# ChainSafe/halo2-verifier

Measured on AMD Instinct MI355X. Metric: proofs verified/sec (BN254, k=14), higher is better.
Workload: dtype u32 limbs (254-bit prime-field integers)

## Files before the change

halo2_verifier_amd/csrc/batch.h:

```cpp
#pragma once
#include "ctx.h"
#include "vkplan.h"
#include <algorithm>
#include <memory>

namespace h2v {

#define H2V_DEV_ST_INVALID_INSTANCES (-40)
#define H2V_DEV_ST_TRANSCRIPT (-30)
#define H2V_DEV_ST_PANIC (-20)
#define H2V_DEV_ST_OPENING (-10)
__device__ __forceinline__ void status_set(int* status, uint32_t p, int dev_code) { atomicMin(&status[p], dev_code); }
__device__ __forceinline__ int status_get(const int* status, uint32_t p) { return __hip_atomic_load(&status[p], __ATOMIC_RELAXED, __HIP_MEMORY_SCOPE_AGENT); }
inline int status_decode(int dev) {
    switch (dev) {
        case 0: return 0;
        case H2V_DEV_ST_INVALID_INSTANCES: return H2V_ERR_INVALID_INSTANCES;
        case H2V_DEV_ST_TRANSCRIPT: return H2V_ERR_TRANSCRIPT;
        case H2V_DEV_ST_PANIC: return H2V_ERR_REFERENCE_PANIC;
        case H2V_DEV_ST_OPENING: return H2V_ERR_OPENING;
        default: return dev;
    }
}

// ... 7 lines not shown
    const Fr* chal; const Fr* mult;
    int* status;
    uint32_t* msm_scal; uint32_t np;
    Fr* shared;
    uint32_t* left_scal;
    const Fr* insteval;
    uint32_t* guard_scal; uint32_t n_guard;
    const VmInstr* code_k[3][FRVM_MAX_STREAMS] = {{nullptr}}; uint32_t n_code_k[3][FRVM_MAX_STREAMS] = {{0}}; uint32_t n_slots_k[3] = {0, 0, 0};
    uint32_t streams = 0;
    int force_streams = 0, force_lds_kb = 0;
};

struct InstEvalArgs {
    const uint8_t* inst; uint32_t ninst;
    const Fr* chal; uint32_t x_chal;
    uint32_t n, k;
    uint32_t base, len;
    Fr w_start, omega, omega_step, omega_step_inv, n_inv;
    Fr* out;
    int* status;
};
int instance_eval_enqueue(hipStream_t s, const InstEvalArgs& a);

inline uint32_t stream_words_for(size_t stream_len, int transcript) {
    const uint32_t words = (uint32_t)((stream_len + 7) / 8);
    const uint32_t blockw = transcript == H2V_TRANSCRIPT_KECCAK256 ? 17 : 16;
    return (words + blockw) / blockw * blockw;
}
struct StageArgs {
    uint32_t n;
    const Plan* plan; const PlanDevice* pd;
    const uint8_t* proofs; const uint8_t* inst;
    G1A* pts; G1A* phi; uint8_t* ycanon; int* status;
    unsigned long long* words; uint32_t stream_words;
    Fr* chal;
};

int decompress_begin_enqueue(hipStream_t s, const StageArgs& g);
int decompress_range_enqueue(hipStream_t s, const StageArgs& g, uint32_t p0, uint32_t p1);
int decompress_finish_enqueue(hipStream_t s, const StageArgs& g);
int transcript_stage_enqueue(hipStream_t s, const StageArgs& g);
size_t multipliers_scratch(uint32_t n_tail, uint32_t groups);
int multipliers_enqueue(hipStream_t s, const uint8_t* d_tail, uint32_t n_tail, uint32_t n, uint32_t groups, Fr* d_mult, Fr* d_scratch);
size_t ragged_multipliers_tiles(uint32_t n);
int ragged_multipliers_enqueue(hipStream_t s, const uint8_t* d_tail, const uint8_t* d_last, uint32_t n, Fr* d_mult, Fr* d_tile_prod, uint32_t* d_tile_words);
int leg_weights_enqueue(hipStream_t s, const uint8_t* d_tail, const Fr* d_mult, const uint32_t* d_off, uint32_t gs, uint32_t groups, uint32_t* d_weights, uint32_t* d_legs);
int gather_multipliers_enqueue(hipStream_t s, const Fr* d_src, const uint32_t* d_idx, uint32_t n, Fr* d_out);
int frvm_enqueue(hipStream_t s, const FrvmArgs& a, uint32_t n_slots);
int fold_shared_enqueue(hipStream_t s, const Fr* d_shared, uint32_t n, uint32_t np, uint32_t n_shared, uint32_t groups, uint32_t* d_msm_scal);
int fold_shared_offsets_enqueue(hipStream_t s, const Fr* d_shared, uint32_t n, uint32_t np, uint32_t n_shared, uint32_t groups, const uint32_t* d_off, uint32_t* d_msm_scal);
struct FoldRange {
    const Fr* shared;
    uint32_t n, n_shared;
    uint32_t first, count;
    uint32_t out, pad;
};
int fold_shared_ranges_enqueue(hipStream_t s, const FoldRange* d_ranges, uint32_t n_ranges, uint32_t max_shared, uint32_t* d_out);

struct Recheck {
    MsmWorkspace ws;
    DevBuf<FoldRange> ranges;
    DevBuf<uint32_t> fold;
    DevBuf<G1J> acc;
    DevBuf<uint32_t> ok;
// ... 104 lines not shown
```

halo2_verifier_amd/csrc/batch.hip:

```cpp
#include "../../include/h2v.h"
#include "batch.h"
#include <string.h>
#include <algorithm>
#include <utility>
#include <stdio.h>

using namespace h2v;

namespace h2v {

struct BatchSizes {
    uint32_t stream_words;
    size_t proofs, inst, pts, ycanon, words, chal, mult, slots, msm_scal, shared, left_scal, insteval, guard_scal, acc, results;
    uint32_t ws_terms, ws_problems, ws_per_problem;
};
BatchSizes batch_sizes(const Plan& pl, size_t N, size_t G, size_t largest) {
    BatchSizes z;
    z.stream_words = stream_words_for(pl.stream.size(), pl.opts.transcript);
    z.proofs = N * pl.proof_len;
    z.inst = N * (size_t)pl.n_instance_values * 32;
    z.pts = N * pl.n_points + pl.n_shared;
    z.ycanon = N * pl.n_points * 32;
    z.words = (size_t)z.stream_words * N;
    z.chal = (size_t)pl.squeeze_at.size() * N;
    z.mult = N;
    z.slots = (size_t)std::max(std::max(pl.n_slots, pl.n_slots_k[0]), std::max(pl.n_slots_k[1], pl.n_slots_k[2])) * N;
    z.msm_scal = (N * pl.n_points + G * pl.n_shared) * 8;
    z.shared = (size_t)pl.n_shared * N;
    z.left_scal = N * pl.n_points * 8;
    z.insteval = N * pl.inst_queries.size();
    z.guard_scal = N * pl.guard_term_order.size() * 8;
    z.acc = 2 * G;
    z.results = ResultsLayout{G, N}.total();
    z.ws_terms = (uint32_t)(2 * (N * pl.n_points + G * pl.n_shared));
    z.ws_problems = (uint32_t)(2 * G);
    z.ws_per_problem = (uint32_t)(largest * pl.n_points + pl.n_shared);
    return z;
}

int ensure_buffers(h2v_batch* b, const Plan& pl) {
    const size_t N = b->max_proofs, G = b->groups;
    size_t largest = (N + G - 1) / G;
    if (ragged(b)) { largest = 0; for (size_t g = 0; g < G; ++g) largest = std::max<size_t>(largest, b->group_off[g + 1] - b->group_off[g]); }
    const BatchSizes z = batch_sizes(pl, N, G, largest);
    int rc;
    if ((rc = b->proofs.reserve(z.proofs)) || (rc = b->inst.reserve(z.inst)) || (rc = b->pts.reserve(z.pts)) || (rc = b->phi.reserve(z.pts)) ||
// ... 265 lines not shown
    return 0;
}

int launch_impl(h2v_batch* b, int with_pairing, const Fr* ext_mult, const uint32_t* ext_idx) {
    int rc;
    if ((rc = require_stage(b, BatchStage::Uploaded, "h2v_batch_launch"))) return rc;
    StageCommit commit{b};
    h2v_ctx* ctx = b->ctx;
    H2V_HIP_CHECK(hipSetDevice(ctx->device));
    PlanDevice* pd = b->plan;
    const Plan& pl = pd->host;
    hipStream_t s = b->stream;
    uint32_t n = b->n;
    const uint32_t G = b->groups;
    if ((rc = join_tail(b))) return rc;
    int ev = 0;
    auto mark = [&]() { if (b->profiling >= 2) hipEventRecord(b->ev[ev], s); ++ev; };
    mark();
    const StageArgs g = stage_args(b);
    const bool run_decompress = !(b->stage == BatchStage::Uploaded && b->decompressed);
    const ResultsLayout L{G, n};
    if (run_decompress && n) H2V_HIP_CHECK(hipMemsetAsync(b->fold_failed, 0, L.total() - L.fold_failed(), s));
    else H2V_HIP_CHECK(hipMemsetAsync(b->fold_failed, 0, 4 * (size_t)G, s));
    if (run_decompress && n && ((rc = decompress_finish_enqueue(s, g)) || (rc = decompress_range_enqueue(s, g, 0, n)))) return rc;
    mark();
    if ((rc = transcript_stage_enqueue(s, g))) return rc;
    MsmProblems pr;
    for (uint32_t g = 0; g < G; ++g)
        channel_problems(pr, b, pl, group_first(b, g), (uint32_t)group_count(b, g), b->acc.p + 2 * g, b->msm_scal.p + ((size_t)n * pl.n_points + (size_t)g * pl.n_shared) * 8, n ? pl.n_shared : 0);
    b->ws.tune = ctx->tuning;
    if (n) {
        if (ext_mult) { b->mult_of_draws = false; if ((rc = gather_multipliers_enqueue(s, ext_mult, ext_idx, n, b->mult.p))) return rc; }
        else if (!b->mult_of_draws) { if ((rc = draw_multipliers_enqueue(b))) return rc; b->mult_of_draws = true; }
        if (!(pl.left_term_order.size() == 1 && !pl.left_term_order[0].first)) H2V_HIP_CHECK(hipMemsetAsync(b->left_scal.p, 0, (size_t)n * pl.n_points * 32, s));
    }
    mark();
    FrvmArgs a{pd->code.p, (uint32_t)pl.code.size(), pd->consts.p, b->slots.p, n, b->proofs.p, pl.proof_len, pd->scalar_offsets.p, b->inst.p, pl.n_instance_values,
               b->chal.p, b->mult.p, b->status, b->msm_scal.p, pl.n_points, b->shared.p, b->left_scal.p, b->insteval.p, b->guard_scal.p, (uint32_t)pl.guard_term_order.size()};
    if (n && pl.wide_instances) {
        Fr step = pl.omega;
        for (int i = 0; i < 8; ++i) step = step.sqr();
        const Fr step_inv = step.inv();
        for (size_t q = 0; q < pl.inst_queries.size(); ++q) {
            InstEvalArgs ia{b->inst.p, pl.n_instance_values, b->chal.p, pl.x_chal, n, pl.domain_k, pl.inst_queries[q].base, pl.inst_queries[q].len,
                            pl.inst_queries[q].w_start, pl.omega, step, step_inv, pl.n_inv, b->insteval.p + q * (size_t)n, b->status};
            if ((rc = instance_eval_enqueue(s, ia))) return rc;
        }
    }
    a.force_streams = ctx->tuning.frvm_streams; a.force_lds_kb = ctx->tuning.frvm_lds_kb;
// ... 408 lines not shown
```

halo2_verifier_amd/csrc/verify_kernels.hip:

```cpp
#include "../../include/h2v.h"
#include "batch.h"
#include <atomic>

namespace h2v {

#define K_DECOMPRESS_LDS_WORDS 2560
__global__ void __launch_bounds__(64, 4) k_decompress(const uint8_t* __restrict__ proofs, uint32_t proof_len, const uint32_t* __restrict__ point_offsets,
                                                   uint32_t np, uint32_t n_main_points, uint32_t n, G1A* __restrict__ pts, G1A* __restrict__ phi, uint8_t* __restrict__ ycanon,
                                                   int* __restrict__ status) {
    const uint32_t t_raw = blockIdx.x * blockDim.x + threadIdx.x;
    const uint32_t t = min(t_raw, n * np - 1);
    uint32_t p = t / np, slot = t % np;
    const uint4* src = reinterpret_cast<const uint4*>(proofs + (size_t)p * proof_len + point_offsets[slot]);
    const uint4 lo = src[0], hi = src[1];
    uint32_t w[8] = {lo.x, lo.y, lo.z, lo.w, hi.x, hi.y, hi.z, hi.w};
    const bool is_inf = (w[7] >> 24) & G1_FLAG_IDENTITY, sign = (w[7] >> 24) & G1_FLAG_SIGN;
    w[7] &= 0x3fffffffu;
    G1A a = G1A::identity();
    bool ok = !Fq::geq_p(w);
    uint32_t yraw[8] = {0, 0, 0, 0, 0, 0, 0, 0};
    if (ok) {
        const Fq x = Fq::from_raw(w);
        if (is_inf) ok = false;
        else {
            const Fq three = {{FqParams::ONE(0), FqParams::ONE(1), FqParams::ONE(2), FqParams::ONE(3), FqParams::ONE(4), FqParams::ONE(5), FqParams::ONE(6), FqParams::ONE(7), FqParams::ONE(8)}};
            const Fq rhs = x.sqr() * x + (three + three + three);
            Fq y = fq_sqrt_candidate_loop_w3(rhs);
            if (y.sqr() != rhs) ok = false;
            else {
                y.to_raw(yraw);
                uint32_t nz = 0;
#pragma unroll
// ... 20 lines not shown
    for (int i = 0; i < 18; ++i) { const uint32_t k = i * 64 + lane; if (k < live * 18) dp[k] = out_lds[k]; }
    __syncthreads();
    a.x = g1_beta_times(a.x);
#pragma unroll
    for (int i = 0; i < 9; ++i) out_lds[lane * 18 + i] = av[i];
    __syncthreads();
    dp = reinterpret_cast<uint32_t*>(phi + t0);
#pragma unroll
    for (int i = 0; i < 18; ++i) { const uint32_t k = i * 64 + lane; if (k < live * 18) dp[k] = out_lds[k]; }
    __syncthreads();
#pragma unroll
    for (int i = 0; i < 8; ++i) out_lds[lane * 8 + i] = yraw[i];
    __syncthreads();
    uint32_t* dy = reinterpret_cast<uint32_t*>(ycanon + (size_t)t0 * 32);
#pragma unroll
    for (int i = 0; i < 8; ++i) { const uint32_t k = i * 64 + lane; if (k < live * 8) dy[k] = out_lds[k]; }
}

__global__ void __launch_bounds__(256) k_check_scalars(const uint8_t* __restrict__ proofs, uint32_t proof_len, const uint32_t* __restrict__ scalar_offsets,
                                                       uint32_t ns, const uint8_t* __restrict__ inst, uint32_t ninst, uint32_t n, int* __restrict__ status) {
    uint32_t t = blockIdx.x * blockDim.x + threadIdx.x;
    uint32_t per = ns + ninst;
    if (t >= n * per) return;
    uint32_t p = t / per, i = t % per;
    const uint8_t* b = i < ns ? proofs + (size_t)p * proof_len + scalar_offsets[i] : inst + ((size_t)p * ninst + (i - ns)) * 32;
    const uint32_t top = ((uintptr_t)b & 3u) == 0 ? *reinterpret_cast<const uint32_t*>(b + 28)
                                                  : (uint32_t)b[28] | ((uint32_t)b[29] << 8) | ((uint32_t)b[30] << 16) | ((uint32_t)b[31] << 24);
    if (top < FrParams::P(7)) return;
    uint32_t raw[8];
    for (int j = 0; j < 8; ++j) raw[j] = (uint32_t)b[4 * j] | ((uint32_t)b[4 * j + 1] << 8) | ((uint32_t)b[4 * j + 2] << 16) | ((uint32_t)b[4 * j + 3] << 24);
    if (Fr::geq_p(raw)) status_set(status, p, i < ns ? H2V_DEV_ST_TRANSCRIPT : H2V_DEV_ST_INVALID_INSTANCES);
}

#define STREAM_PROOFS_PER_BLOCK 8u
__global__ void __launch_bounds__(256) k_stream_build(const TranscriptSrc* __restrict__ stream, uint32_t stream_len, const uint8_t* __restrict__ proofs,
                                                      uint32_t proof_len, const uint8_t* __restrict__ ycanon, uint32_t np, const uint8_t* __restrict__ inst,
                                                      uint32_t ninst, uint32_t n, uint32_t stream_words, unsigned long long* __restrict__ words) {
    const uint32_t p0 = blockIdx.x * STREAM_PROOFS_PER_BLOCK, p1 = min(n, p0 + STREAM_PROOFS_PER_BLOCK);
    for (uint32_t w = threadIdx.x; w < stream_words; w += blockDim.x) {
        uint32_t kind[8], value[8], off[8];
#pragma unroll
        for (uint32_t b = 0; b < 8; ++b) {
            const uint32_t pos = w * 8 + b, q = pos < stream_len ? pos : stream_len - 1;
            const TranscriptSrc sd = stream[q];
            kind[b] = pos < stream_len ? sd.kind : (uint32_t)TranscriptSrc::CONST;
            value[b] = pos < stream_len ? sd.value : 0u;
            off[b] = kind[b] == TranscriptSrc::CONST ? 0u : sd.offset;
        }
        auto is_data = [](uint32_t k) { return k != TranscriptSrc::CONST; };
        auto src_of = [](uint32_t k) { return k == TranscriptSrc::PROOF_MASKED ? (uint32_t)TranscriptSrc::PROOF : k; };
        uint32_t la = 0;
        while (la < 8 && is_data(kind[la]) && src_of(kind[la]) == src_of(kind[0]) && off[la] == off[0] + la) ++la;
        uint32_t sb = la;
        unsigned long long cbytes = 0;
// ... 127 lines not shown
        }
        const uint32_t rem = len - last_blk * 128;
        __syncthreads();
#pragma unroll
        for (uint32_t j = 0; j < 4; ++j) {
            unsigned long long w = pf_blk == last_blk ? pf[j] : words[(size_t)last_blk * 16 + 4 * r + j];
            const uint32_t lo = 8 * (4 * r + j);
            if (lo >= rem) w = 0;
            else if (lo + 8 > rem) w &= (1ULL << (8 * (rem - lo))) - 1;
            msg[4 * r + j] = w;
        }
        __syncthreads();
        unsigned long long c0 = h0, c1 = h1;
        blake2b_compress_quad(c0, c1, msg, sig, len, true, r);
        dig[q * 8 + r] = c0; dig[q * 8 + 4 + r] = c1;
    }
    __syncthreads();
    for (uint32_t q = r; q < n_squeeze; q += 4) {
        uint32_t w32[16];
#pragma unroll
        for (int i = 0; i < 8; ++i) { const unsigned long long v = dig[q * 8 + i]; w32[2 * i] = (uint32_t)v; w32[2 * i + 1] = (uint32_t)(v >> 32); }
        const Fr c = Fr::from_uniform_words(w32);
        if (p_raw < n) chal[(size_t)q * n + p] = c;
    }
}

__device__ __forceinline__ unsigned long long rotl64(unsigned long long x, int c) { return c ? (x << c) | (x >> (64 - c)) : x; }
__constant__ unsigned long long KECCAK_RC[24] = {
    0x0000000000000001ULL, 0x0000000000008082ULL, 0x800000000000808aULL, 0x8000000080008000ULL, 0x000000000000808bULL, 0x0000000080000001ULL,
    0x8000000080008081ULL, 0x8000000000008009ULL, 0x000000000000008aULL, 0x0000000000000088ULL, 0x0000000080008009ULL, 0x000000008000000aULL,
    0x000000008000808bULL, 0x800000000000008bULL, 0x8000000000008089ULL, 0x8000000000008003ULL, 0x8000000000008002ULL, 0x8000000000000080ULL,
    0x000000000000800aULL, 0x800000008000000aULL, 0x8000000080008081ULL, 0x8000000000008080ULL, 0x0000000080000001ULL, 0x8000000080008008ULL};
__device__ __noinline__ void keccak_f1600(unsigned long long a[25]) {
    const int ROT[25] = {0, 1, 62, 28, 27, 36, 44, 6, 55, 20, 3, 10, 43, 25, 39, 41, 45, 15, 21, 8, 18, 2, 61, 56, 14};
    for (int r = 0; r < 24; ++r) {
        unsigned long long c[5], b[25];
#pragma unroll
        for (int x = 0; x < 5; ++x) c[x] = a[x] ^ a[x + 5] ^ a[x + 10] ^ a[x + 15] ^ a[x + 20];
#pragma unroll
        for (int x = 0; x < 5; ++x) {
            unsigned long long d = c[(x + 4) % 5] ^ rotl64(c[(x + 1) % 5], 1);
#pragma unroll
            for (int y = 0; y < 5; ++y) a[x + 5 * y] ^= d;
        }
#pragma unroll
        for (int x = 0; x < 5; ++x)
// ... 393 lines not shown
    red[t] = acc;
    __syncthreads();
    for (uint32_t d = 32; d > 0; d >>= 1) {
        if (t < d) red[t] = red[t] + red[t + d];
        __syncthreads();
    }
    if (t == 0) {
        uint32_t raw[8]; red[0].to_raw(raw);
        uint32_t* dst = out + ((size_t)rg.out + j) * 8;
        for (int i = 0; i < 8; ++i) dst[i] = raw[i];
    }
}

int decompress_begin_enqueue(hipStream_t s, const StageArgs& g) {
    if (g.n) H2V_HIP_CHECK(hipMemsetAsync(g.status, 0, sizeof(int) * g.n, s));
    return 0;
}
int decompress_range_enqueue(hipStream_t s, const StageArgs& g, uint32_t p0, uint32_t p1) {
    if (p1 <= p0) return 0;
    const Plan& pl = *g.plan;
    const uint32_t m = p1 - p0, tp = m * pl.n_points;
    if (!tp) return 0;
    hipLaunchKernelGGL(k_decompress, dim3((tp + 63) / 64), dim3(64), 0, s, g.proofs + (size_t)p0 * pl.proof_len, pl.proof_len, g.pd->point_offsets.p, pl.n_points, pl.n_main_points, m,
                       g.pts + (size_t)p0 * pl.n_points, g.phi + (size_t)p0 * pl.n_points, g.ycanon + (size_t)p0 * pl.n_points * 32, g.status + p0);
    H2V_HIP_CHECK(hipGetLastError());
    return 0;
}
int decompress_finish_enqueue(hipStream_t s, const StageArgs& g) {
    const Plan& pl = *g.plan;
    const uint32_t ts = g.n * (pl.n_scalars + pl.n_instance_values);
    if (ts) hipLaunchKernelGGL(k_check_scalars, dim3((ts + 255) / 256), dim3(256), 0, s, g.proofs, pl.proof_len, g.pd->scalar_offsets.p, pl.n_scalars, g.inst, pl.n_instance_values, g.n, g.status);
    H2V_HIP_CHECK(hipGetLastError());
    return 0;
}
int transcript_stage_enqueue(hipStream_t s, const StageArgs& g) {
    const uint32_t n = g.n;
    if (!n) return 0;
    const Plan& pl = *g.plan;
    uint32_t stream_len = (uint32_t)pl.stream.size();
    uint32_t n_words = g.stream_words;
    const bool keccak = pl.opts.transcript == H2V_TRANSCRIPT_KECCAK256;
    const uint32_t nsq = (uint32_t)pl.squeeze_at.size();
    const size_t lds = ((size_t)16 * TR4_MSG_STRIDE + (size_t)16 * nsq * 8) * 8;
    if (!keccak && lds > 60 * 1024) { set_last_error("transcript: too many challenges for one workgroup's LDS"); return H2V_ERR_UNSUPPORTED; }
    hipLaunchKernelGGL(k_stream_build, dim3((n + STREAM_PROOFS_PER_BLOCK - 1) / STREAM_PROOFS_PER_BLOCK), dim3(256), 0, s, g.pd->stream.p, stream_len, g.proofs, pl.proof_len, g.ycanon, pl.n_points, g.inst,
                       pl.n_instance_values, n, n_words, g.words);
    if (keccak)
        hipLaunchKernelGGL(k_transcript_keccak, dim3((n + 63) / 64), dim3(64), 0, s, g.words, n_words, g.pd->squeeze_at.p, nsq, n, g.chal);
    else
        hipLaunchKernelGGL(k_transcript, dim3((n + 15) / 16), dim3(64), lds, s, g.words, n_words, g.pd->squeeze_at.p, nsq, n, g.chal);
    H2V_HIP_CHECK(hipGetLastError());
    return 0;
}
size_t multipliers_scratch(uint32_t n_tail, uint32_t groups) { return (size_t)groups * ((n_tail / groups + MULT_TILE - 1) / MULT_TILE); }
int multipliers_enqueue(hipStream_t s, const uint8_t* d_tail, uint32_t n_tail, uint32_t n, uint32_t groups, Fr* d_mult, Fr* d_scratch) {
    const uint32_t nt = n_tail / groups, ng = n / groups, tiles = (nt + MULT_TILE - 1) / MULT_TILE;
    if (!tiles || !ng) return 0;
    if (tiles > 65535u * 1024u || groups > 65535u) { set_last_error("multipliers: too many draws or groups"); return H2V_ERR_BAD_ARGUMENT; }
    hipLaunchKernelGGL(k_mult_tiles, dim3(tiles, groups), dim3(MULT_TILE), 0, s, d_tail, nt, ng, tiles, d_mult, d_scratch);
    if (tiles > 1) {
        hipLaunchKernelGGL(k_mult_scan_tiles, dim3(groups), dim3(1024), 0, s, d_scratch, tiles);
        hipLaunchKernelGGL(k_mult_apply, dim3((ng + MULT_TILE - 1) / MULT_TILE, groups), dim3(MULT_TILE), 0, s, d_mult, ng, tiles, (const Fr*)d_scratch);
    }
    H2V_HIP_CHECK(hipGetLastError());
    return 0;
}
size_t ragged_multipliers_tiles(uint32_t n) { return ((size_t)n + MULT_TILE - 1) / MULT_TILE; }
int ragged_multipliers_enqueue(hipStream_t s, const uint8_t* d_tail, const uint8_t* d_last, uint32_t n, Fr* d_mult, Fr* d_tile_prod, uint32_t* d_tile_words) {
    const uint32_t tiles = (uint32_t)ragged_multipliers_tiles(n);
    if (!tiles) return 0;
    uint32_t* tile_closed = d_tile_words; uint32_t* open_from = d_tile_words + tiles;
    hipLaunchKernelGGL(k_seg_mult_tiles, dim3(tiles), dim3(MULT_TILE), 0, s, d_tail, d_last, n, d_mult, d_tile_prod, tile_closed, open_from);
    if (tiles > 1) {
// ... 75 lines not shown
```

halo2_verifier_amd/csrc/vkplan.h:

```cpp
#pragma once
#include "ctx.h"
#include <map>
#include <mutex>

namespace h2v {

static const uint8_t COL_INSTANCE = 254, COL_FIXED = 255;
struct ColumnH { uint32_t index; uint8_t type; };
struct QueryH { ColumnH column; int32_t rotation; };
struct TermH { uint16_t coeff_idx; std::vector<std::pair<uint32_t, uint32_t>> factors; };
struct ExprH { uint32_t num_vars = 0; std::vector<TermH> terms; };
struct LookupH { std::vector<ExprH> input, table; };
struct ShuffleH { std::vector<ExprH> input, shuffle; };

struct VkHost {
    uint32_t k = 0, cs_degree = 0;
    std::vector<G1A> fixed_commitments, permutation_commitments;
    Fr transcript_repr;
    uint32_t num_fixed_columns = 0, num_advice_columns = 0, num_instance_columns = 0, num_selectors = 0, num_challenges = 0;
    std::vector<uint8_t> advice_column_phase, challenge_phase;
    std::vector<uint32_t> num_advice_queries;
    std::vector<QueryH> advice_queries, instance_queries, fixed_queries;
    std::vector<ColumnH> permutation_columns;
    std::vector<ExprH> gates;
// ... 16 lines not shown
    OP_INV = 6,
    OP_POW = 7,
    OP_SQRN = 8,
    OP_LOAD_SCALAR = 9,
    OP_LOAD_INST = 10,
    OP_LOAD_CHAL = 11,
    OP_LOAD_MULT = 12,
    OP_STORE_MSM = 13,
    OP_STORE_SHARED = 14,
    OP_STORE_LEFT = 15,
    OP_LOAD_INSTEVAL = 16,
    OP_STORE_GUARD = 17,
    OP_BARRIER = 18,
};
struct VmInstr { uint32_t op, d, a, b; };
#define FRVM_MAX_STREAMS 4
#define VM_CONST_OPERAND 0x80000000u

struct TranscriptSrc {
    enum Kind : uint8_t { CONST = 0, PROOF = 1, PROOF_MASKED = 2, YCOORD = 3, INSTANCE = 4 };
    uint8_t kind; uint8_t value; uint32_t offset;
};

struct PlanOptions { int multiopen = 0; int transcript = 0; int circuit_instances = 1; bool guard_terms = false; int instance_kernel_threshold = 0; };

struct Plan {
    PlanOptions opts;
    double dag_work = 0, dag_critical_path = 0, makespan_k[3] = {0, 0, 0};
    uint32_t n_points = 0, n_scalars = 0, proof_len = 0;
    std::vector<uint32_t> point_offsets, scalar_offsets;
    uint32_t n_main_points = 0;
    uint32_t slot_h1 = 0, slot_h2 = 0;
    uint32_t opening_offset = 0;
    std::vector<std::pair<uint8_t, uint32_t>> left_term_order;
    std::vector<TranscriptSrc> stream;
    std::vector<uint32_t> squeeze_at;
    std::vector<uint32_t> squeeze_order;
    uint32_t n_challenges = 0;
    uint32_t n_user_challenges = 0;
    std::vector<VmInstr> code;
    std::vector<Fr> consts;
    uint32_t n_slots = 0;
    std::vector<VmInstr> code_k[3][FRVM_MAX_STREAMS];
    uint32_t n_slots_k[3] = {0, 0, 0};
    uint32_t n_shared = 0;
    std::vector<G1A> shared_bases;
    std::vector<std::pair<uint8_t, uint32_t>> right_term_order;
    std::vector<std::pair<uint8_t, uint32_t>> guard_term_order;
    std::vector<size_t> col_lens;
    uint32_t n_instance_values = 0;
    struct InstQuery { uint32_t base, len; Fr w_start; };
    bool wide_instances = false;
    std::vector<InstQuery> inst_queries;
    uint32_t x_chal = 0, domain_k = 0;
    Fr omega, n_inv;
};
int compile_plan(const VkHost& vk, const ParamsHost& params, const std::vector<size_t>& col_lens, PlanOptions opts, Plan& out, std::string& err);

struct PlanDevice {
    Plan host;
    DevBuf<VmInstr> code;
    DevBuf<VmInstr> code_k[3][FRVM_MAX_STREAMS];
    DevBuf<Fr> consts;
    DevBuf<TranscriptSrc> stream;
    DevBuf<uint32_t> squeeze_at;
    DevBuf<uint32_t> point_offsets;
    DevBuf<uint32_t> scalar_offsets;
    DevBuf<G1A> shared_bases, shared_phi;
    int pins = 0;
    uint64_t last_use = 0;
    int upload();
};

#define H2V_MAX_CACHED_PLANS 32
struct VkDevice {
    VkHost vk;
    std::map<std::vector<size_t>, PlanDevice*> plans;
    uint64_t clock = 0;
    std::mutex mu;
};
int ctx_get_plan(h2v_ctx* ctx, const std::vector<size_t>& col_lens, PlanDevice** out, bool guard_terms = false);
void ctx_put_plan(h2v_ctx* ctx, PlanDevice* pd);
struct PlanPin {
    h2v_ctx* ctx; PlanDevice* pd = nullptr;
    explicit PlanPin(h2v_ctx* c) : ctx(c) {}
    PlanPin(const PlanPin&) = delete;
    PlanPin& operator=(const PlanPin&) = delete;
// ... 7 lines not shown
```

halo2_verifier_amd/csrc/vkplan.hip:

```cpp
#include "../../include/h2v.h"
#include "ctx.h"
#include "vkplan.h"
#include <algorithm>
#include <array>
#include <set>
#include <stdio.h>
#include <stdlib.h>
#include <string.h>

namespace h2v {

namespace {
struct Reader {
    const uint8_t* d; size_t n, pos = 0; bool ok = true;
    Reader(const uint8_t* p, size_t len) : d(p), n(len) {}
    const uint8_t* take(size_t k) {
        static const uint8_t zeros[128] = {0};
        if (pos + k > n) { ok = false; return zeros; }
        const uint8_t* r = d + pos; pos += k; return r;
    }
    uint8_t u8() { return *take(1); }
    uint16_t u16() { const uint8_t* b = take(2); return (uint16_t)((b[0] << 8) | b[1]); }
    uint32_t u32() { const uint8_t* b = take(4); return ((uint32_t)b[0] << 24) | ((uint32_t)b[1] << 16) | ((uint32_t)b[2] << 8) | b[3]; }
    int32_t i32() { return (int32_t)u32(); }
// ... 967 lines not shown
    const Inverses iv = invert(b, vk, s, dom, col_lens, plan.wide_instances, c, z_diff_0);
    const std::vector<std::vector<Val>> instance_evals = instance_evaluations(b, vk, s, dom, iv, plan);
    bool panic = false;
    const Val h_eval = expected_h_eval(b, vk, s, dom, c, iv, inst, vkl, instance_evals, panic);
    if (panic) { err = "the VK makes the reference panic (empty expression polynomial or out-of-range index)"; return H2V_ERR_REFERENCE_PANIC; }
    const Val mult = b.load_mult();
    plan.shared_bases.clear();
    for (const G1A& g : vk.fixed_commitments) plan.shared_bases.push_back(g);
    for (const G1A& g : vk.permutation_commitments) plan.shared_bases.push_back(g);
    plan.shared_bases.push_back(params.g);
    if (s.gwc) plan.shared_bases.back().y = plan.shared_bases.back().y.neg();
    plan.n_shared = (uint32_t)plan.shared_bases.size();
    Scalars out(plan.n_points, plan.n_shared, opts.guard_terms && s.gwc);
    if (s.gwc) gwc_scalars(b, c, op, point_of, h_eval, vkl, out);
    else shplonk_scalars(b, dom, c, op, point_of, iv, h_eval, vkl, plan, out);
    plan.right_term_order = out.right_order; plan.left_term_order = out.left_order; plan.guard_term_order = out.guard_order;
    for (uint32_t i = 0; i < plan.n_points; ++i) b.store_msm(out.msm[i] == NONE ? b.zero() : b.mul(out.msm[i], mult), i);
    for (uint32_t j = 0; j < plan.n_shared; ++j) b.store_shared(out.shared[j] == NONE ? b.zero() : b.mul(out.shared[j], mult), j);
    for (uint32_t i = 0; i < plan.n_points; ++i) if (out.left[i] != NONE) b.store_left(b.mul(out.left[i], mult), i);
    b.emit(plan.code, plan.n_slots);
    for (int K = 2; K <= FRVM_MAX_STREAMS; ++K) { b.emit_streams(K, plan.code_k[K - 2], plan.n_slots_k[K - 2]); plan.makespan_k[K - 2] = b.makespan_k; }
    b.dag_costs(plan.dag_work, plan.dag_critical_path);
    plan.consts = b.consts;
    return 0;
}

template <class T> static int upload_vec(const std::vector<T>& v, DevBuf<T>& d) {
    int rc;
    if ((rc = d.alloc(v.size()))) return rc;
    if (!v.empty()) H2V_HIP_CHECK(hipMemcpy(d.p, v.data(), v.size() * sizeof(T), hipMemcpyHostToDevice));
    return 0;
}
int PlanDevice::upload() {
    int rc;
    if ((rc = upload_vec(host.code, code))) return rc;
    for (int k = 0; k < 3; ++k) for (int q = 0; q < k + 2; ++q) if ((rc = upload_vec(host.code_k[k][q], code_k[k][q]))) return rc;
    if ((rc = upload_vec(host.consts, consts))) return rc;
    if ((rc = upload_vec(host.stream, stream))) return rc;
    if ((rc = upload_vec(host.squeeze_at, squeeze_at))) return rc;
    if ((rc = upload_vec(host.point_offsets, point_offsets))) return rc;
    if ((rc = upload_vec(host.scalar_offsets, scalar_offsets))) return rc;
    if ((rc = upload_vec(host.shared_bases, shared_bases))) return rc;
    std::vector<G1A> phi;
    for (const G1A& b : host.shared_bases) phi.push_back(g1_phi(b));
    if ((rc = upload_vec(phi, shared_phi))) return rc;
    return 0;
}

int ctx_load_vk(h2v_ctx* ctx, const uint8_t* vk, size_t vk_len, int vk_format) {
    VkDevice* v = new VkDevice();
    std::string err;
    if (!vk_from_bytes(vk, vk_len, vk_format, v->vk, err)) { set_last_error("VerifyingKey: " + err); delete v; return H2V_ERR_FORMAT; }
    if (v->vk.k != ctx->params.k) { set_last_error("VerifyingKey: k differs from ParamsKZG.k"); delete v; return H2V_ERR_BAD_ARGUMENT; }
    ctx->vk = v;
    return 0;
}
size_t ctx_total_instance_columns(const h2v_ctx* ctx) { return ctx->vk ? (size_t)ctx->circuit_instances * ctx->vk->vk.num_instance_columns : 0; }
void ctx_release_vk(h2v_ctx* ctx) {
    if (!ctx->vk) return;
    for (auto& kv : ctx->vk->plans) delete kv.second;
    delete ctx->vk;
// ... 41 lines not shown
```

Baseline: 11.89 million.

## Hash Blake2b transcript directly from proof bytes via precompiled word descriptors

For Blake2b transcripts, the transcript kernel now builds each 64-bit message word from the proof, y-coordinate and instance buffers. It uses per-word descriptors compiled at plan time, so the packed-words buffer and the kernel that filled it are no longer needed. The scalar range check is folded into the decompress kernel as extra blocks, which removes a launch. This cuts global memory traffic and kernel launches, at the cost of unaligned gathers, a slow per-byte fallback, and more complex descriptor logic.

```diff
diff --git a/halo2_verifier_amd/csrc/batch.h b/halo2_verifier_amd/csrc/batch.h
--- a/halo2_verifier_amd/csrc/batch.h
+++ b/halo2_verifier_amd/csrc/batch.h
@@ -53,11 +53,6 @@
 };
 int instance_eval_enqueue(hipStream_t s, const InstEvalArgs& a);
 
-inline uint32_t stream_words_for(size_t stream_len, int transcript) {
-    const uint32_t words = (uint32_t)((stream_len + 7) / 8);
-    const uint32_t blockw = transcript == H2V_TRANSCRIPT_KECCAK256 ? 17 : 16;
-    return (words + blockw) / blockw * blockw;
-}
 struct StageArgs {
     uint32_t n;
     const Plan* plan; const PlanDevice* pd;
@@ -71,6 +66,8 @@
 int decompress_range_enqueue(hipStream_t s, const StageArgs& g, uint32_t p0, uint32_t p1);
 int decompress_finish_enqueue(hipStream_t s, const StageArgs& g);
 int transcript_stage_enqueue(hipStream_t s, const StageArgs& g);
+int decompress_checked_enqueue(hipStream_t s, const StageArgs& g);
+int transcript_direct_enqueue(hipStream_t s, const StageArgs& g);
 size_t multipliers_scratch(uint32_t n_tail, uint32_t groups);
 int multipliers_enqueue(hipStream_t s, const uint8_t* d_tail, uint32_t n_tail, uint32_t n, uint32_t groups, Fr* d_mult, Fr* d_scratch);
 size_t ragged_multipliers_tiles(uint32_t n);
diff --git a/halo2_verifier_amd/csrc/batch.hip b/halo2_verifier_amd/csrc/batch.hip
--- a/halo2_verifier_amd/csrc/batch.hip
+++ b/halo2_verifier_amd/csrc/batch.hip
@@ -21,7 +21,7 @@
     z.inst = N * (size_t)pl.n_instance_values * 32;
     z.pts = N * pl.n_points + pl.n_shared;
     z.ycanon = N * pl.n_points * 32;
-    z.words = (size_t)z.stream_words * N;
+    z.words = pl.opts.transcript == H2V_TRANSCRIPT_KECCAK256 ? (size_t)z.stream_words * N : 0;
     z.chal = (size_t)pl.squeeze_at.size() * N;
     z.mult = N;
     z.slots = (size_t)std::max(std::max(pl.n_slots, pl.n_slots_k[0]), std::max(pl.n_slots_k[1], pl.n_slots_k[2])) * N;
@@ -333,9 +333,13 @@
     const ResultsLayout L{G, n};
     if (run_decompress && n) H2V_HIP_CHECK(hipMemsetAsync(b->fold_failed, 0, L.total() - L.fold_failed(), s));
     else H2V_HIP_CHECK(hipMemsetAsync(b->fold_failed, 0, 4 * (size_t)G, s));
-    if (run_decompress && n && ((rc = decompress_finish_enqueue(s, g)) || (rc = decompress_range_enqueue(s, g, 0, n)))) return rc;
+    const bool direct = pl.opts.transcript != H2V_TRANSCRIPT_KECCAK256;
+    if (run_decompress && n) {
+        if (direct) { if ((rc = decompress_checked_enqueue(s, g))) return rc; }
+        else if ((rc = decompress_finish_enqueue(s, g)) || (rc = decompress_range_enqueue(s, g, 0, n))) return rc;
+    }
     mark();
-    if ((rc = transcript_stage_enqueue(s, g))) return rc;
+    if ((rc = direct ? transcript_direct_enqueue(s, g) : transcript_stage_enqueue(s, g))) return rc;
     MsmProblems pr;
     for (uint32_t g = 0; g < G; ++g)
         channel_problems(pr, b, pl, group_first(b, g), (uint32_t)group_count(b, g), b->acc.p + 2 * g, b->msm_scal.p + ((size_t)n * pl.n_points + (size_t)g * pl.n_shared) * 8, n ? pl.n_shared : 0);
diff --git a/halo2_verifier_amd/csrc/verify_kernels.hip b/halo2_verifier_amd/csrc/verify_kernels.hip
--- a/halo2_verifier_amd/csrc/verify_kernels.hip
+++ b/halo2_verifier_amd/csrc/verify_kernels.hip
@@ -5,9 +5,35 @@
 namespace h2v {
 
 #define K_DECOMPRESS_LDS_WORDS 2560
+__device__ __forceinline__ void check_scalar(const uint8_t* __restrict__ proofs, uint32_t proof_len, const uint32_t* __restrict__ scalar_offsets, uint32_t ns,
+                                             const uint8_t* __restrict__ inst, uint32_t ninst, uint32_t p, uint32_t i, int* __restrict__ status) {
+    const uint8_t* b = i < ns ? proofs + (size_t)p * proof_len + scalar_offsets[i] : inst + ((size_t)p * ninst + (i - ns)) * 32;
+    const uint32_t top = ((uintptr_t)b & 3u) == 0 ? *reinterpret_cast<const uint32_t*>(b + 28)
+                                                  : (uint32_t)b[28] | ((uint32_t)b[29] << 8) | ((uint32_t)b[30] << 16) | ((uint32_t)b[31] << 24);
+    if (top < FrParams::P(7)) return;
+    uint32_t raw[8];
+    for (int j = 0; j < 8; ++j) raw[j] = (uint32_t)b[4 * j] | ((uint32_t)b[4 * j + 1] << 8) | ((uint32_t)b[4 * j + 2] << 16) | ((uint32_t)b[4 * j + 3] << 24);
+    if (Fr::geq_p(raw)) status_set(status, p, i < ns ? H2V_DEV_ST_TRANSCRIPT : H2V_DEV_ST_INVALID_INSTANCES);
+}
+#define CHECK_PER_LANE 8u
+#define CHECK_PER_BLOCK (64u * CHECK_PER_LANE)
+struct ScalarCheck {
+    uint32_t point_blocks;
+    uint32_t ns, ninst;
+    const uint32_t* scalar_offsets;
+    const uint8_t* inst;
+};
 __global__ void __launch_bounds__(64, 4) k_decompress(const uint8_t* __restrict__ proofs, uint32_t proof_len, const uint32_t* __restrict__ point_offsets,
                                                    uint32_t np, uint32_t n_main_points, uint32_t n, G1A* __restrict__ pts, G1A* __restrict__ phi, uint8_t* __restrict__ ycanon,
-                                                   int* __restrict__ status) {
+                                                   int* __restrict__ status, const ScalarCheck sc) {
+    if (blockIdx.x >= sc.point_blocks) {
+        const uint32_t per = sc.ns + sc.ninst, total = n * per, t0 = (blockIdx.x - sc.point_blocks) * CHECK_PER_BLOCK + threadIdx.x;
+        for (uint32_t k = 0; k < CHECK_PER_LANE; ++k) {
+            const uint32_t t = t0 + k * 64;
+            if (t < total) check_scalar(proofs, proof_len, sc.scalar_offsets, sc.ns, sc.inst, sc.ninst, t / per, t % per, status);
+        }
+        return;
+    }
     const uint32_t t_raw = blockIdx.x * blockDim.x + threadIdx.x;
     const uint32_t t = min(t_raw, n * np - 1);
     uint32_t p = t / np, slot = t % np;
@@ -74,14 +100,7 @@
     uint32_t t = blockIdx.x * blockDim.x + threadIdx.x;
     uint32_t per = ns + ninst;
     if (t >= n * per) return;
-    uint32_t p = t / per, i = t % per;
-    const uint8_t* b = i < ns ? proofs + (size_t)p * proof_len + scalar_offsets[i] : inst + ((size_t)p * ninst + (i - ns)) * 32;
-    const uint32_t top = ((uintptr_t)b & 3u) == 0 ? *reinterpret_cast<const uint32_t*>(b + 28)
-                                                  : (uint32_t)b[28] | ((uint32_t)b[29] << 8) | ((uint32_t)b[30] << 16) | ((uint32_t)b[31] << 24);
-    if (top < FrParams::P(7)) return;
-    uint32_t raw[8];
-    for (int j = 0; j < 8; ++j) raw[j] = (uint32_t)b[4 * j] | ((uint32_t)b[4 * j + 1] << 8) | ((uint32_t)b[4 * j + 2] << 16) | ((uint32_t)b[4 * j + 3] << 24);
-    if (Fr::geq_p(raw)) status_set(status, p, i < ns ? H2V_DEV_ST_TRANSCRIPT : H2V_DEV_ST_INVALID_INSTANCES);
+    check_scalar(proofs, proof_len, scalar_offsets, ns, inst, ninst, t / per, t % per, status);
 }
 
 #define STREAM_PROOFS_PER_BLOCK 8u
@@ -255,6 +274,123 @@
         for (int i = 0; i < 8; ++i) { const unsigned long long v = dig[q * 8 + i]; w32[2 * i] = (uint32_t)v; w32[2 * i + 1] = (uint32_t)(v >> 32); }
         const Fr c = Fr::from_uniform_words(w32);
         if (p_raw < n) chal[(size_t)q * n + p] = c;
+    }
+}
+
+__device__ __forceinline__ unsigned long long transcript_word_bytes(const TranscriptSrc* __restrict__ stream, uint32_t stream_len, uint32_t pos0, const uint8_t* pb,
+                                                                 const uint8_t* yb, const uint8_t* ib) {
+    unsigned long long v = 0;
+#pragma nounroll
+    for (uint32_t k = 0; k < 8 && pos0 + k < stream_len; ++k) {
+        const TranscriptSrc sd = stream[pos0 + k];
+        const uint8_t* const base = sd.kind == TranscriptSrc::YCOORD ? yb : (sd.kind == TranscriptSrc::INSTANCE ? ib : pb);
+        uint32_t byte = sd.kind == TranscriptSrc::CONST ? sd.value : base[sd.offset];
+        if (sd.kind == TranscriptSrc::PROOF_MASKED) byte &= 0x3f;
+        v |= (unsigned long long)byte << (8 * k);
+    }
+    return v;
+}
+struct TranscriptDirectArgs {
+    const StreamWord* desc; uint32_t n_desc;
+    const TranscriptSrc* stream; uint32_t stream_len;
+    const uint8_t* proofs; const uint8_t* ycanon; const uint8_t* inst;
+    uint32_t proof_len, np, ninst;
+    const uint32_t* squeeze_at; uint32_t n_squeeze;
+    uint32_t n; Fr* chal;
+};
+__global__ void __launch_bounds__(64) k_transcript_direct(const TranscriptDirectArgs g) {
+    extern __shared__ unsigned long long tr_lds[];
+    typedef unsigned long long u64_unaligned __attribute__((aligned(1)));
+    const uint32_t tid = threadIdx.x, r = tid & 3u, pq = tid >> 2, n = g.n, n_squeeze = g.n_squeeze;
+    const uint32_t p_raw = blockIdx.x * 16 + pq, p = p_raw < n ? p_raw : n - 1;
+    const uint8_t* const pb = g.proofs + (size_t)p * g.proof_len;
+    const uint8_t* const yb = g.ycanon + (size_t)p * g.np * 32;
+    const uint8_t* const ib = g.inst + (size_t)p * g.ninst * 32;
+    unsigned long long* msg = tr_lds + pq * TR4_MSG_STRIDE;
+    unsigned long long* dig = tr_lds + 16 * TR4_MSG_STRIDE + (size_t)pq * n_squeeze * 8;
+    uint32_t sig[12];
+#pragma unroll
+    for (int rd = 0; rd < 12; ++rd)
+        sig[rd] = (uint32_t)BLAKE_SIGMA[rd][2 * r] | ((uint32_t)BLAKE_SIGMA[rd][2 * r + 1] << 4) | ((uint32_t)BLAKE_SIGMA[rd][8 + 2 * r] << 8) | ((uint32_t)BLAKE_SIGMA[rd][9 + 2 * r] << 12);
+    const unsigned long long pers0 = 0x72542d326f6c6148ULL, pers1 = 0x7470697263736e61ULL;
+    unsigned long long h0 = BLAKE_IV[r] ^ (r == 0 ? 0x01010040ULL : 0ULL), h1 = BLAKE_IV[4 + r] ^ (r == 2 ? pers0 : (r == 3 ? pers1 : 0ULL));
+    const uint32_t n_blocks = g.n_desc / 16;
+    const unsigned long long at_p = (unsigned long long)p * g.proof_len;
+    const unsigned long long diff_y = (unsigned long long)(g.ycanon - g.proofs) + (unsigned long long)p * g.np * 32 - at_p;
+    const unsigned long long diff_i = (unsigned long long)(g.inst - g.proofs) + (unsigned long long)p * g.ninst * 32 - at_p;
+    auto addr_of = [&](uint32_t code, uint32_t off) -> const u64_unaligned* {
+        return reinterpret_cast<const u64_unaligned*>(g.proofs + (at_p + off + (diff_y & (0ULL - (code & 1u))) + (diff_i & (0ULL - ((code >> 1) & 1u)))));
+    };
+    unsigned long long* const stage = tr_lds + 16 * TR4_MSG_STRIDE + (size_t)16 * n_squeeze * 8;
+    const unsigned long long* const desc64 = reinterpret_cast<const unsigned long long*>(g.desc);
+    static_assert(sizeof(StreamWord) == 32, "four 64-bit words per descriptor: a block's are one word per lane");
+    auto chunk = [&](uint32_t b) -> unsigned long long {
+        return desc64[(size_t)(b < n_blocks ? b : n_blocks - 1) * 64 + tid];
+    };
+    StreamWord dc[4];
+    unsigned long long ra[4], rb[4];
+    auto stage_get = [&]() {
+        const StreamWord* sp = reinterpret_cast<const StreamWord*>(stage) + 4 * r;
+#pragma unroll
+        for (uint32_t j = 0; j < 4; ++j) dc[j] = sp[j];
+    };
+    auto fetch = [&](const StreamWord (&d)[4]) {
+#pragma unroll
+        for (uint32_t j = 0; j < 4; ++j) {
+            const uint32_t c = d[j].ctl;
+            ra[j] = *addr_of(c & 3u, d[j].off_a);
+            rb[j] = *addr_of((c >> 8) & 3u, d[j].off_b);
+        }
+    };
+    auto word = [&](const StreamWord (&d)[4], uint32_t b, uint32_t j) -> unsigned long long {
+        const uint32_t c = d[j].ctl, la = (c >> 4) & 15u, sb = (c >> 12) & 15u;
+        const unsigned long long va = ra[j] >> ((8 * (8 - la)) & 63u), vb = rb[j] << ((8 * sb) & 63u);
+        unsigned long long v = (d[j].cbytes | (la ? va : 0ULL) | (sb < 8 ? vb : 0ULL)) & d[j].keep;
+        if (__builtin_expect(c & STREAM_WORD_SLOW, 0)) v = transcript_word_bytes(g.stream, g.stream_len, (b * 16 + 4 * r + j) * 8, pb, yb, ib);
+        return v;
+    };
+    uint32_t blk = 0;
+    stage[tid] = chunk(0);
+    __syncthreads();
+    stage_get();
+    fetch(dc);
+    unsigned long long pd = chunk(1);
+    for (uint32_t q = 0; q < n_squeeze; ++q) {
+        const uint32_t len = g.squeeze_at[q];
+        const uint32_t last_blk = (len - 1) / 128;
+        for (; blk < last_blk; ++blk) {
+            __syncthreads();
+#pragma unroll
+            for (uint32_t j = 0; j < 4; ++j) msg[4 * r + j] = word(dc, blk, j);
+            stage[tid] = pd;
+            __syncthreads();
+            stage_get();
+            fetch(dc);
+            pd = chunk(blk + 2);
+            blake2b_compress_quad(h0, h1, msg, sig, (unsigned long long)(blk + 1) * 128, false, r);
+        }
+        const uint32_t rem = len - last_blk * 128;
+        __syncthreads();
+#pragma unroll
+        for (uint32_t j = 0; j < 4; ++j) {
+            unsigned long long w = word(dc, last_blk, j);
+            const uint32_t lo = 8 * (4 * r + j);
+            if (lo >= rem) w = 0;
+            else if (lo + 8 > rem) w &= (1ULL << (8 * (rem - lo))) - 1;
+            msg[4 * r + j] = w;
+        }
+        __syncthreads();
+        unsigned long long c0 = h0, c1 = h1;
+        blake2b_compress_quad(c0, c1, msg, sig, len, true, r);
+        dig[q * 8 + r] = c0; dig[q * 8 + 4 + r] = c1;
+    }
+    __syncthreads();
+    for (uint32_t q = r; q < n_squeeze; q += 4) {
+        uint32_t w32[16];
+#pragma unroll
+        for (int i = 0; i < 8; ++i) { const unsigned long long v = dig[q * 8 + i]; w32[2 * i] = (uint32_t)v; w32[2 * i + 1] = (uint32_t)(v >> 32); }
+        const Fr c = Fr::from_uniform_words(w32);
+        if (p_raw < n) g.chal[(size_t)q * n + p] = c;
     }
 }
 
@@ -694,7 +830,19 @@
     const uint32_t m = p1 - p0, tp = m * pl.n_points;
     if (!tp) return 0;
     hipLaunchKernelGGL(k_decompress, dim3((tp + 63) / 64), dim3(64), 0, s, g.proofs + (size_t)p0 * pl.proof_len, pl.proof_len, g.pd->point_offsets.p, pl.n_points, pl.n_main_points, m,
-                       g.pts + (size_t)p0 * pl.n_points, g.phi + (size_t)p0 * pl.n_points, g.ycanon + (size_t)p0 * pl.n_points * 32, g.status + p0);
+                       g.pts + (size_t)p0 * pl.n_points, g.phi + (size_t)p0 * pl.n_points, g.ycanon + (size_t)p0 * pl.n_points * 32, g.status + p0,
+                       ScalarCheck{(tp + 63) / 64, 0, 0, nullptr, nullptr});
+    H2V_HIP_CHECK(hipGetLastError());
+    return 0;
+}
+int decompress_checked_enqueue(hipStream_t s, const StageArgs& g) {
+    const Plan& pl = *g.plan;
+    const uint64_t tp = (uint64_t)g.n * pl.n_points, ts = (uint64_t)g.n * ((uint64_t)pl.n_scalars + pl.n_instance_values);
+    if (tp > 0xffffffffull - 64 || ts > 0xffffffffull - CHECK_PER_BLOCK) { set_last_error("decompress: too many points or scalars for one launch"); return H2V_ERR_UNSUPPORTED; }
+    const uint32_t point_blocks = (uint32_t)((tp + 63) / 64), check_blocks = (uint32_t)((ts + CHECK_PER_BLOCK - 1) / CHECK_PER_BLOCK);
+    if (!(point_blocks + check_blocks)) return 0;
+    hipLaunchKernelGGL(k_decompress, dim3(point_blocks + check_blocks), dim3(64), 0, s, g.proofs, pl.proof_len, g.pd->point_offsets.p, pl.n_points, pl.n_main_points, g.n,
+                       g.pts, g.phi, g.ycanon, g.status, ScalarCheck{point_blocks, pl.n_scalars, pl.n_instance_values, g.pd->scalar_offsets.p, g.inst});
     H2V_HIP_CHECK(hipGetLastError());
     return 0;
 }
@@ -721,6 +869,23 @@
         hipLaunchKernelGGL(k_transcript_keccak, dim3((n + 63) / 64), dim3(64), 0, s, g.words, n_words, g.pd->squeeze_at.p, nsq, n, g.chal);
     else
         hipLaunchKernelGGL(k_transcript, dim3((n + 15) / 16), dim3(64), lds, s, g.words, n_words, g.pd->squeeze_at.p, nsq, n, g.chal);
+    H2V_HIP_CHECK(hipGetLastError());
+    return 0;
+}
+int transcript_direct_enqueue(hipStream_t s, const StageArgs& g) {
+    const uint32_t n = g.n;
+    if (!n) return 0;
+    const Plan& pl = *g.plan;
+    if (pl.opts.transcript == H2V_TRANSCRIPT_KECCAK256) { set_last_error("transcript: the direct form is Blake2b's"); return H2V_ERR_UNSUPPORTED; }
+    const uint32_t nsq = (uint32_t)pl.squeeze_at.size(), stream_len = (uint32_t)pl.stream.size(), n_desc = (uint32_t)pl.stream_words.size();
+    const size_t lds = ((size_t)16 * TR4_MSG_STRIDE + (size_t)16 * nsq * 8) * 8;
+    if (lds > 60 * 1024) { set_last_error("transcript: too many challenges for one workgroup's LDS"); return H2V_ERR_UNSUPPORTED; }
+    bool ok = n_desc % 16 == 0 && (size_t)n_desc * 8 > stream_len && stream_len >= 1 && g.pd->stream_words.p && n_desc == stream_words_for(stream_len, pl.opts.transcript);
+    for (uint32_t q = 0; ok && q < nsq; ++q) ok = pl.squeeze_at[q] >= 1 && pl.squeeze_at[q] <= stream_len && (q == 0 || pl.squeeze_at[q] >= pl.squeeze_at[q - 1]);
+    if (!ok) { set_last_error("transcript: the plan's word descriptors or squeeze positions do not match its stream"); return H2V_ERR_BAD_ARGUMENT; }
+    TranscriptDirectArgs a{g.pd->stream_words.p, n_desc, g.pd->stream.p, stream_len, g.proofs, g.ycanon, g.inst, pl.proof_len, pl.n_points, pl.n_instance_values,
+                           g.pd->squeeze_at.p, nsq, n, g.chal};
+    hipLaunchKernelGGL(k_transcript_direct, dim3((n + 15) / 16), dim3(64), lds + 64 * 8, s, a);
     H2V_HIP_CHECK(hipGetLastError());
     return 0;
 }
diff --git a/halo2_verifier_amd/csrc/vkplan.h b/halo2_verifier_amd/csrc/vkplan.h
--- a/halo2_verifier_amd/csrc/vkplan.h
+++ b/halo2_verifier_amd/csrc/vkplan.h
@@ -62,6 +62,19 @@
     uint8_t kind; uint8_t value; uint32_t offset;
 };
 
+struct StreamWord {
+    unsigned long long cbytes;
+    unsigned long long keep;
+    uint32_t off_a, off_b, ctl, pad;
+};
+#define STREAM_WORD_SLOW 0x80000000u
+
+inline uint32_t stream_words_for(size_t stream_len, int transcript) {
+    const uint32_t words = (uint32_t)((stream_len + 7) / 8);
+    const uint32_t blockw = transcript == H2V_TRANSCRIPT_KECCAK256 ? 17 : 16;
+    return (words + blockw) / blockw * blockw;
+}
+
 struct PlanOptions { int multiopen = 0; int transcript = 0; int circuit_instances = 1; bool guard_terms = false; int instance_kernel_threshold = 0; };
 
 struct Plan {
@@ -74,6 +87,7 @@
     uint32_t opening_offset = 0;
     std::vector<std::pair<uint8_t, uint32_t>> left_term_order;
     std::vector<TranscriptSrc> stream;
+    std::vector<StreamWord> stream_words;
     std::vector<uint32_t> squeeze_at;
     std::vector<uint32_t> squeeze_order;
     uint32_t n_challenges = 0;
@@ -95,6 +109,48 @@
     uint32_t x_chal = 0, domain_k = 0;
     Fr omega, n_inv;
 };
+inline void compile_stream_words(Plan& plan) {
+    const size_t stream_len = plan.stream.size();
+    const uint32_t n_words = stream_words_for(stream_len, plan.opts.transcript);
+    auto is_data = [](uint32_t k) { return k != TranscriptSrc::CONST; };
+    auto src_of = [](uint32_t k) { return k == TranscriptSrc::PROOF_MASKED ? (uint32_t)TranscriptSrc::PROOF : k; };
+    auto per_of = [&](uint32_t src) -> uint64_t {
+        return src == TranscriptSrc::YCOORD ? (uint64_t)plan.n_points * 32 : (src == TranscriptSrc::INSTANCE ? (uint64_t)plan.n_instance_values * 32 : (uint64_t)plan.proof_len);
+    };
+    plan.stream_words.resize(n_words);
+    for (uint32_t w = 0; w < n_words; ++w) {
+        uint32_t kind[8], value[8], off[8];
+        for (uint32_t b = 0; b < 8; ++b) {
+            const size_t pos = (size_t)w * 8 + b;
+            kind[b] = pos < stream_len ? plan.stream[pos].kind : (uint32_t)TranscriptSrc::CONST;
+            value[b] = pos < stream_len ? plan.stream[pos].value : 0u;
+            off[b] = kind[b] == TranscriptSrc::CONST ? 0u : plan.stream[pos].offset;
+        }
+        uint32_t la = 0;
+        while (la < 8 && is_data(kind[la]) && src_of(kind[la]) == src_of(kind[0]) && off[la] == off[0] + la) ++la;
+        uint32_t sb = la;
+        unsigned long long cbytes = 0;
+        while (sb < 8 && !is_data(kind[sb])) { cbytes |= (unsigned long long)value[sb] << (8 * sb); ++sb; }
+        bool fits = true;
+        for (uint32_t b = sb; b < 8; ++b) fits = fits && is_data(kind[b]) && src_of(kind[b]) == src_of(kind[sb]) && off[b] == off[sb] + (b - sb);
+        if (la > 0 && la < 8 && off[0] < 8 - la) fits = false;
+        unsigned long long keep = ~0ULL;
+        for (uint32_t b = 0; b < 8; ++b) if (kind[b] == TranscriptSrc::PROOF_MASKED) keep &= ~(0xc0ULL << (8 * b));
+        auto code_of = [](uint32_t src) { return src == TranscriptSrc::YCOORD ? 1u : (src == TranscriptSrc::INSTANCE ? 2u : 0u); };
+        StreamWord d{0, ~0ULL, 0, 0, 0, 0};
+        uint32_t code_a = 0, code_b = 0;
+        if (la) { d.off_a = off[0] + la - 8; code_a = code_of(src_of(kind[0])); }
+        if (sb < 8) { d.off_b = off[sb]; code_b = code_of(src_of(kind[sb])); }
+        if (!la) { d.off_a = d.off_b; code_a = code_b; }
+        if (sb == 8) { d.off_b = d.off_a; code_b = code_a; }
+        const uint64_t per[3] = {per_of(TranscriptSrc::PROOF), per_of(TranscriptSrc::YCOORD), per_of(TranscriptSrc::INSTANCE)};
+        if ((uint64_t)d.off_a + 8 > per[code_a] || (uint64_t)d.off_b + 8 > per[code_b]) fits = false;
+        if (fits) { d.cbytes = cbytes; d.keep = keep; d.ctl = code_a | (la << 4) | (code_b << 8) | (sb << 12); }
+        else d = StreamWord{0, ~0ULL, 0, 0, STREAM_WORD_SLOW | (8u << 12), 0};
+        plan.stream_words[w] = d;
+    }
+}
+
 int compile_plan(const VkHost& vk, const ParamsHost& params, const std::vector<size_t>& col_lens, PlanOptions opts, Plan& out, std::string& err);
 
 struct PlanDevice {
@@ -103,6 +159,7 @@
     DevBuf<VmInstr> code_k[3][FRVM_MAX_STREAMS];
     DevBuf<Fr> consts;
     DevBuf<TranscriptSrc> stream;
+    DevBuf<StreamWord> stream_words;
     DevBuf<uint32_t> squeeze_at;
     DevBuf<uint32_t> point_offsets;
     DevBuf<uint32_t> scalar_offsets;
diff --git a/halo2_verifier_amd/csrc/vkplan.hip b/halo2_verifier_amd/csrc/vkplan.hip
--- a/halo2_verifier_amd/csrc/vkplan.hip
+++ b/halo2_verifier_amd/csrc/vkplan.hip
@@ -1013,6 +1013,7 @@
     for (int K = 2; K <= FRVM_MAX_STREAMS; ++K) { b.emit_streams(K, plan.code_k[K - 2], plan.n_slots_k[K - 2]); plan.makespan_k[K - 2] = b.makespan_k; }
     b.dag_costs(plan.dag_work, plan.dag_critical_path);
     plan.consts = b.consts;
+    compile_stream_words(plan);
     return 0;
 }
 
@@ -1028,6 +1029,7 @@
     for (int k = 0; k < 3; ++k) for (int q = 0; q < k + 2; ++q) if ((rc = upload_vec(host.code_k[k][q], code_k[k][q]))) return rc;
     if ((rc = upload_vec(host.consts, consts))) return rc;
     if ((rc = upload_vec(host.stream, stream))) return rc;
+    if ((rc = upload_vec(host.stream_words, stream_words))) return rc;
     if ((rc = upload_vec(host.squeeze_at, squeeze_at))) return rc;
     if ((rc = upload_vec(host.point_offsets, point_offsets))) return rc;
     if ((rc = upload_vec(host.scalar_offsets, scalar_offsets))) return rc;
```

Result: no change. 11.91 million (median of 2 runs) (+0.1%).
